# Boese0601/RC-MVSNet

Hardware: AMD Instinct MI355X
Metric: ref-scenes/sec (DTU 3-view 512x640, D=48/32/8) (higher is better)
Workload: dtype f32; 1 GPU; BASELINE configs[1]: CascadeMVSNet_eval.forward, DTU-shaped 3 views 512x640, D=(48,32,8), batch 1 per GPU, fp32, random-init seeded weights; views=3, height=512, width=640, parallelism=scene-per-gpu x1, ranks=1, procs_per_gpu=1, rccl_ranks=0

## Files before the change

rc_mvsnet_amd/_lib.py:

```python
import ast
import ctypes
import os
import re
import subprocess

_HERE = os.path.dirname(os.path.abspath(__file__))
LIB_PATH = os.path.join(_HERE, "librcmvs_hip.so")
CSRC = os.path.join(_HERE, "csrc")
HEADER = os.path.join(os.path.dirname(_HERE), "include", "rcmvs.h")
EXT_HEADERS = (os.path.join(CSRC, "pc_register.h"), os.path.join(CSRC, "view_select.h"), os.path.join(CSRC, "undistort.h"),
               os.path.join(CSRC, "tsdf_mesh.h"), os.path.join(CSRC, "tsdf_sparse.h"), os.path.join(CSRC, "mesh_clean.h"),
               os.path.join(CSRC, "mesh_decimate.h"), os.path.join(CSRC, "mesh_holes.h"))

_lib = None


class RcmvsError(RuntimeError):
    pass


_CTYPES = {"int": ctypes.c_int, "float": ctypes.c_float, "double": ctypes.c_double, "long long": ctypes.c_longlong}


def _const_expr(text):
    def ev(node):
        if isinstance(node, ast.Constant) and type(node.value) is int:
            return node.value
        if isinstance(node, ast.BinOp) and isinstance(node.op, ast.LShift):
            return ev(node.left) << ev(node.right)
        raise ValueError(text)
    return ev(ast.parse(text.strip(), mode="eval").body)


def _ctype(decl, what, c_type):
    if c_type not in _CTYPES:
        raise RcmvsError(f"{HEADER}: `{decl}`: {what} type `{c_type}` is outside the ABI's types ({', '.join(_CTYPES)}, pointers)")
    return _CTYPES[c_type]


def parse_header(text):
    text = re.sub(r"/\*.*?\*/|//[^\n]*", " ", text, flags=re.S)
    signatures, restypes, constants, code = {}, {}, {}, []
    for line in text.splitlines():
        if not line.lstrip().startswith("#"):
            code.append(line)
            continue
        m = re.match(r"\s*#\s*define\s+(RCMVS_\w+)\s+(\S.*)", line)
        if m:
            try:
                value = _const_expr(m.group(2))
            except (ValueError, SyntaxError):
                raise RcmvsError(f"{HEADER}: `{line.strip()}`: not an integer expression of literals, << and parentheses") from None
            if m.group(1) in constants:
                raise RcmvsError(f"{HEADER}: {m.group(1)} is defined twice")
            constants[m.group(1)] = value
    for decl in re.sub(r'extern\s+"C"\s*\{', " ", "\n".join(code)).split(";"):
        decl = " ".join(decl.split())
        if "rcmvs_" not in decl:
            continue
        m = re.fullmatch(r"([\w\s*]+?)\s*\b(rcmvs_\w+)\s*\(([^()]*)\)", decl)
        if not m:
            raise RcmvsError(f"{HEADER}: `{decl}` is not a complete `<type> rcmvs_name(<parameters>);` declaration")
        ret, name, params = m.group(1), m.group(2), m.group(3).strip()
        if name in signatures:
            raise RcmvsError(f"{HEADER}: {name} is declared twice")
# ... 117 lines not shown
```

rc_mvsnet_amd/casmvsnet.py:

```python
import os

FP16_PAIR_DEFAULT = True
ONE_BY_ONE_MFMA = os.environ.get("RCMVS_1X1_MFMA", "1") != "0"
HEAD_PAIR = os.environ.get("RCMVS_HEAD_PAIR", "1") != "0"
CONV11_PROB = int(os.environ.get("RCMVS_CONV11_PROB", "1"))
CONV_TILE = os.environ.get("RCMVS_CONV_TILE", "1") != "0"
CONV_STEM = os.environ.get("RCMVS_CONV_STEM", "1") != "0"
CONV_PAIR = os.environ.get("RCMVS_CONV_PAIR", "1") != "0"
DEEP_PAIR = os.environ.get("RCMVS_DEEP_PAIR", "1") != "0"

import torch
import torch.nn as nn
import torch.nn.functional as F

from . import ops
from ._lib import RcmvsError


def _nhwc(x):
    x = x.contiguous().float()
    return ops.rgb_to_nhwc4(x) if x.shape[1] == 3 else ops.to_channels_last(x)


def _param(mod, name):
    p = mod._parameters.get(name)
    return p if p is not None else getattr(mod, name)


def _packed_of(module, make):
    w = module.conv.weight
    key = (w.data_ptr(), w._version, str(w.device))
    c = module.__dict__.get("_rcmvs_pack")
    if c is None or c[0] != key:
        c = module.__dict__["_rcmvs_pack"] = (key, make(w.detach()))
    return c[1]


def _affine_of(m):
    if getattr(m, "gn", None) is not None:
        raise RcmvsError(f"{type(m).__name__}: GroupNorm blocks are not provided (the reference builds every block with norm='batch_norm')")
    if m.bn is not None:
        return _bn_fold(m.bn)
    b = m.conv.bias
    if b is None:
        return None, None
    return torch.ones_like(b, dtype=torch.float32), b.detach().float().contiguous()


def _same2(v, n):
    return tuple(v) == (n, n)


def _conv2d_block_cl(m, t):
    conv = m.conv
    K = conv.kernel_size[0]
    st = conv.stride[0]
    if (not _same2(conv.kernel_size, K) or K not in (1, 3, 5) or not _same2(conv.padding, K // 2) or not _same2(conv.stride, st)
            or st not in (1, 2) or not _same2(conv.dilation, 1) or conv.groups != 1 or conv.padding_mode != "zeros"):
        raise RcmvsError(f"Conv2d: only square 1x1 / 3x3 / 5x5 kernels with 'same' zero padding, stride 1 or 2, no dilation or groups "
                         f"(the layers of models/modules.py) run on the HIP path; got {conv}")
# ... 105 lines not shown
                self.out_channels.append(b)
        elif num_stage == 3:
            self.inner1 = nn.Conv2d(b * 2, final_chs, 1, bias=True)
            self.inner2 = nn.Conv2d(b * 1, final_chs, 1, bias=True)
            self.out2 = nn.Conv2d(final_chs, b * 2, 3, padding=1, bias=False)
            self.out3 = nn.Conv2d(final_chs, b, 3, padding=1, bias=False)
            self.out_channels += [b * 2, b]
        elif num_stage == 2:
            self.inner1 = nn.Conv2d(b * 2, final_chs, 1, bias=True)
            self.out2 = nn.Conv2d(final_chs, b, 3, padding=1, bias=False)
            self.out_channels.append(b)

    def hip_plan(self):
        sub = self._modules
        mods = [m for seq in ("conv0", "conv1", "conv2") for m in sub[seq]._modules.values()]
        tens = []
        for m in mods:
            cv, bn = m._modules["conv"], m._modules["bn"]
            bb = bn._buffers
            tens += [_param(cv, "weight"), _param(bn, "weight"), _param(bn, "bias"), bb["running_mean"], bb["running_var"], bb["num_batches_tracked"]]
        unet = self.arch_mode == "unet"
        heads = ["out1"] + (["out2", "out3"] if unet else ["inner1", "out2", "inner2", "out3"])
        extra = [t for n in heads if n in sub for t in (_param(sub[n], "weight"), getattr(sub[n], "bias", None)) if t is not None]
        key = tuple((t.data_ptr(), t._version) for t in tens + extra)
        if getattr(self, "_plan", None) is None or key != self._plan_key:
            plan = {}
            names = ["conv0.0", "conv0.1", "conv1.0", "conv1.1", "conv1.2", "conv2.0", "conv2.1", "conv2.2"]
            for n, m in zip(names, mods):
                pad_to = 4 if m.conv.in_channels == 3 else None
                w = m.conv.weight
                if tuple(w.shape) in ((8, 8, 3, 3), (16, 16, 3, 3), (32, 32, 3, 3)) and m.stride == 1:
                    w3 = w.detach().new_zeros(w.shape[0], w.shape[1], 3, 3, 3)
                    w3[:, :, 1] = w.detach()
                    plan[n] = ("mfma3d", ops.pack_conv3d_weight(w3)) + _bn_fold(m.bn)
                    continue
                if tuple(w.shape) in ((32, 16, 5, 5), (16, 8, 5, 5)) and m.stride == 2:
                    w3 = self._w3(self._w5s2(w.detach())).contiguous()
                    plan[n] = ("s2d_mfma3d", ops.pack_conv3d_weight(w3)) + _bn_fold(m.bn)
                    continue
                plan[n] = (ops.pack_conv2d_weight(w, pad_in_to=pad_to),) + _bn_fold(m.bn) + (m.stride,)
            m11, m12 = mods[3], mods[4]
            if CONV_PAIR and all(tuple(m.conv.weight.shape) == (16, 16, 3, 3) and m.stride == 1 for m in (m11, m12)):
                plan["pair1"] = (ops.pack_conv2d_pair(m11.conv.weight, m12.conv.weight),) + _bn_fold(m11.bn) + _bn_fold(m12.bn)
            m00, m01 = mods[0], mods[1]
            if CONV_STEM and tuple(m00.conv.weight.shape) == (8, 3, 3, 3) and tuple(m01.conv.weight.shape) == (8, 8, 3, 3) and m00.stride == 1 and m01.stride == 1:
                plan["stem"] = (plan["conv0.0"][0],) + _bn_fold(m00.bn) + (ops.pack_conv2d_stem(m01.conv.weight),) + _bn_fold(m01.bn)
            m10 = mods[2]
            if CONV_TILE and tuple(m10.conv.weight.shape) == (16, 8, 5, 5) and m10.stride == 2:
                plan["tile10"] = (ops.pack_conv2d_tile(self._w5s2(m10.conv.weight.detach()).contiguous()),) + _bn_fold(m10.bn)
            for n, m in (("conv2.1", mods[6]), ("conv2.2", mods[7])):
                if CONV_TILE and tuple(m.conv.weight.shape) == (32, 32, 3, 3) and m.stride == 1:
                    plan["tile:" + n] = (ops.pack_conv2d_tile(m.conv.weight),) + _bn_fold(m.bn)
            plan["out1"] = ops.pack_conv2d_weight(self.out1.weight)
            if unet:
                for n in ("out2", "out3")[:self.num_stage - 1]:
                    plan[n] = ops.pack_conv3d_weight(self._w3(getattr(self, n).weight.detach()))
            elif self.num_stage >= 2:
                plan["inner1"] = (ops.pack_conv2d_weight(self.inner1.weight), self.inner1.bias.detach().float().contiguous())
                if tuple(self.out2.weight.shape) == (16, 32, 3, 3):
                    w3 = self.out2.weight.detach().new_zeros(16, 32, 3, 3, 3)
                    w3[:, :, 1] = self.out2.weight.detach()
                    plan["out2"] = ("mfma3d", ops.pack_conv3d_weight(w3))
                    if CONV_TILE:
                        plan["out2t"] = ops.pack_conv2d_tile(self.out2.weight)
                else:
                    plan["out2"] = ops.pack_conv2d_weight(self.out2.weight)
            if self.num_stage == 3 and not unet:
                plan["inner2"] = (ops.pack_conv2d_weight(self.inner2.weight), self.inner2.bias.detach().float().contiguous())
                plan["out3"] = ops.pack_conv2d_weight(self.out3.weight)
                plan["fuse_out3"] = tuple(self.inner2.weight.shape[:2]) == (32, 8) and tuple(self.out3.weight.shape[:2]) == (8, 32)
                if plan["fuse_out3"]:
                    plan["fold_out3"] = ops.pack_fpn_folded(self.inner2.weight, self.inner2.bias, self.out3.weight)
                    if os.environ.get("RCMVS_FPN_MFMA", "1") != "0":
                        plan["fold_out3"] = ops.pack_fpn_folded_mfma(plan["fold_out3"])
            self._plan, self._plan_key = plan, key
        return self._plan

    def forward_cl(self, x, lazy=False):
        p = self.hip_plan()

        def cbr(t, n):
            if "tile:" + n in p and not ops._CONV_IMPL:
                img, sc, sh = p["tile:" + n]
                return ops.conv2d_tile(t, img, sc, sh, relu=True)
            if p[n][0] == "mfma3d":
                _, w3, sc, sh = p[n]
                return ops.conv3d(t.unsqueeze(1), w3, sc, sh, relu=True).squeeze(1)
            if p[n][0] == "s2d_mfma3d":
                if t.shape[1] % 2 or t.shape[2] % 2:
                    raise RcmvsError(f"FeatureNet: image height and width must be multiples of 4 (got a {t.shape[1]}x{t.shape[2]} map "
                                     "at the second stride-2 layer), as the reference's three-level pyramid requires")
                _, w3, sc, sh = p[n]
                if ops._CONV_IMPL:
                    return ops.conv3d(self._s2d(t).contiguous().unsqueeze(1), w3, sc, sh, relu=True).squeeze(1)
                return ops.conv2d_s2d(t, w3, sc, sh, relu=True)
            w, sc, sh, stride = p[n]
            return ops.conv2d(t, w, sc, sh, stride=stride, relu=True)

        w00 = p["conv0.0"][0] if len(p["conv0.0"]) == 4 else None
        if "stem" in p and not ops._CONV_IMPL:
            c0 = ops.conv2d_stem(x.contiguous().float(), *p["stem"])
        else:
            c0 = None
        if c0 is not None:
            pass
        elif w00 is not None and w00.ci == 4 and w00.co == 8 and w00.k == 3 and p["conv0.0"][3] == 1 and not ops._CONV_IMPL:
            w, sc, sh, _ = p["conv0.0"]
            c0 = cbr(ops.conv2d_rgb(x.contiguous().float(), w, sc, sh, relu=True), "conv0.1")
        else:
            c0 = cbr(cbr(ops.rgb_to_nhwc4(x.contiguous().float()), "conv0.0"), "conv0.1")
        if "tile10" in p and not ops._CONV_IMPL and c0.shape[1] % 2 == 0 and c0.shape[2] % 2 == 0:
            c10 = ops.conv2d_tile(c0, p["tile10"][0], p["tile10"][1], p["tile10"][2], relu=True, s2d=True)
        else:
            c10 = cbr(c0, "conv1.0")
        if "pair1" in p and not ops._CONV_IMPL:
            c1 = ops.conv2d_pair(c10, *p["pair1"])
        else:
            c1 = cbr(cbr(c10, "conv1.1"), "conv1.2")
        c2 = cbr(cbr(cbr(c1, "conv2.0"), "conv2.1"), "conv2.2")
        def out1(bound=None, t=c2):
            if tuple(self.out1.weight.shape) == (32, 32, 1, 1) and (bound is not None or ONE_BY_ONE_MFMA):
                return ops.conv1x1(t, p["out1"], ysq_absmax=bound, mfma=ONE_BY_ONE_MFMA), bound is not None
            return ops.conv2d(t, p["out1"]), False
        out = {"stage1": out1}
        plain = lambda f: (lambda bound=None: (f(), False))
        if self.arch_mode == "unet":
            one = lambda t, n: ops.conv3d(t.unsqueeze(1), p[n]).squeeze(1)
            if self.num_stage >= 2:
                intra = self.deconv1.forward_cl(c1, c2)
                out["stage2"] = plain(lambda t=intra: one(t, "out2"))
            if self.num_stage == 3:
                intra = self.deconv2.forward_cl(c0, intra)
                out["stage3"] = plain(lambda t=intra: one(t, "out3"))
            return out if lazy else {k: f()[0] for k, f in out.items()}
        if self.num_stage >= 2:
            intra = ops.conv2d(c1, p["inner1"][0], None, p["inner1"][1], up_add=c2)
            if isinstance(p["out2"], tuple):
                def out2(bound=None, t=intra):
                    keep = bound is not None and not ops._CONV_IMPL
                    if "out2t" in p and not ops._CONV_IMPL:
                        return ops.conv2d_tile(t, p["out2t"], ysq_absmax=bound), keep
                    return ops.conv3d(t.unsqueeze(1), p["out2"][1], y_absmax=bound if keep else None, y_absmax_square=keep).squeeze(1), keep
                out["stage2"] = out2
            else:
                out["stage2"] = plain(lambda t=intra: ops.conv2d(t, p["out2"]))
        if self.num_stage == 3:
            if p.get("fuse_out3") and c0.shape[1] % 2 == 0 and c0.shape[2] % 2 == 0:
                if p.get("fold_out3") is not None:
                    out["stage3"] = (lambda bound=None, a=c0, b=intra: (ops.fpn_out_folded(a, b, p["fold_out3"], ysq_absmax=bound), bound is not None))
                else:
                    out["stage3"] = plain(lambda a=c0, b=intra: ops.fpn_out_fused(a, b, p["inner2"][0], p["inner2"][1], p["out3"]))
            else:
                intra = ops.conv2d(c0, p["inner2"][0], None, p["inner2"][1], up_add=intra)
                out["stage3"] = plain(lambda t=intra: ops.conv2d(t, p["out3"]))
        return out if lazy else {k: f()[0] for k, f in out.items()}

    @staticmethod
    def _w3(w):
        p = (3 - w.shape[-1]) // 2
        return F.pad(w.unsqueeze(2), (p, p, p, p, 1, 1))

    @staticmethod
    def _w5s2(w):
        Co, Ci = w.shape[:2]
        w6 = F.pad(w, (0, 1, 0, 1))
        return w6.reshape(Co, Ci, 3, 2, 3, 2).permute(0, 3, 5, 1, 2, 4).reshape(Co, 4 * Ci, 3, 3)

    @staticmethod
    def _s2d(x):
        N, H, W, C = x.shape
        return x.reshape(N, H // 2, 2, W // 2, 2, C).permute(0, 1, 3, 2, 4, 5).reshape(N, H // 2, W // 2, 4 * C)

    def forward_train_cl(self, x, segments=1):
        from .train_ops import ConvPlainFn, conv_bn_train_w
        if self.arch_mode != "fpn":
            raise RcmvsError("FeatureNet(arch_mode='unet'): the train-mode HIP path covers the shipped 'fpn' pyramid only (the one-plane form of "
                             "its transposed convs would put the discarded plane into the batch statistics)")
        N, _, H, W = x.shape
        if H % 4 or W % 4:
            raise RcmvsError("FeatureNet (training): image height and width must be multiples of 4")
        t = F.pad(x.permute(0, 2, 3, 1), (0, 5)).contiguous()

        def cbr(t, m):
            w = m.conv.weight
            if m.stride == 2:
                t, w = self._s2d(t), self._w5s2(w)
            return conv_bn_train_w(self._w3(w), m.bn, t.unsqueeze(1), relu=True, segments=segments).squeeze(1)

        def plain(t, conv):
# ... 266 lines not shown
            out = {"depth": depth, "photometric_confidence": conf}
            if self.train_variant:
                out["volume_feature_no_ref"] = ops.warp_noref(f_cl, small_cl, rot, trans, planes, D, square_first=True)
            return out
        if _hip_training(self, *features, depth_values):
            from . import train_ops
            f_cl = torch.stack([f.float().permute(0, 2, 3, 1) for f in features], dim=1).contiguous()
            res = ops.WarpVarianceFn.apply(f_cl, rot, trans, planes, D, small_cl)
            var, noref = res if self.train_variant else (res, None)
            x8 = cost_regularization.features_cl_train(var)
            depth, conf = train_ops.ProbDepthHeadFn.apply(x8, cost_regularization.prob.weight, planes)
            out = {"depth": depth, "photometric_confidence": conf}
            if self.train_variant:
                out["volume_feature_no_ref"] = noref
            return out
        _unsupported(self, *features, depth_values)


class _CascadeBase(nn.Module):
    TRAIN_VARIANT = False

    def __init__(self, refine=False, ndepths=[48, 32, 8], depth_interals_ratio=[4, 2, 1], share_cr=False,
                 grad_method="detach", arch_mode="fpn", cr_base_chs=[8, 8, 8]):
        super().__init__()
        if refine:
            raise NotImplementedError("refine=True: the reference's RefineNet is not runnable (models/modules.py:511 calls F.cat)")
        self.refine = refine
        self.share_cr = share_cr
        self.ndepths = ndepths
        self.depth_interals_ratio = depth_interals_ratio
        self.grad_method = grad_method
        self.arch_mode = arch_mode
        self.cr_base_chs = cr_base_chs
        self.num_stage = len(ndepths)
        assert len(ndepths) == len(depth_interals_ratio)
        self.stage_infos = {"stage1": {"scale": 4.0}, "stage2": {"scale": 2.0}, "stage3": {"scale": 1.0}}
        self.feature = FeatureNet(base_channels=8, stride=4, num_stage=self.num_stage, arch_mode=self.arch_mode)
        if self.share_cr:
            self.cost_regularization = CostRegNet(in_channels=self.feature.out_channels, base_channels=8)
        else:
            self.cost_regularization = nn.ModuleList([CostRegNet(in_channels=self.feature.out_channels[i],
                                                                 base_channels=self.cr_base_chs[i])
                                                      for i in range(self.num_stage)])
        self.DepthNet = DepthNet(self.TRAIN_VARIANT)

    def _cr(self, s):
        return self.cost_regularization if self.share_cr else self.cost_regularization[s]

    def _forward_hip(self, imgs, proj_matrices, depth_values, features=None, homographies=None):
        B, V, _, H, W = imgs.shape
        imgs = imgs.float()
        depth_values = depth_values.contiguous().float()
        feats_cl = None
        if features is None:
            feats_cl = self.feature.forward_cl(imgs.reshape(B * V, 3, H, W), lazy=True)
        outputs = {}
        depth = None
        bounds = None
        need_fill = False
        pair = getattr(self, "fp16_pair", None)
        if pair is None:
            pair = FP16_PAIR_DEFAULT if os.environ.get("RCMVS_FP16_PAIR") is None else os.environ["RCMVS_FP16_PAIR"] == "1"
        if pair and B == 1:
            bounds = getattr(self, "_pair_bounds", None)
            if getattr(self, "_is_replica", False):
                bounds = torch.zeros(self.num_stage, CostRegNet.BOUND_ROWS, ops.ABSMAX_FLOATS, device=imgs.device, dtype=torch.float32)
            elif bounds is None or bounds.device != imgs.device:
                bounds = self._pair_bounds = torch.zeros(self.num_stage, CostRegNet.BOUND_ROWS, ops.ABSMAX_FLOATS, device=imgs.device, dtype=torch.float32)
            else:
                need_fill = True
        if homographies is None:
            if self.num_stage <= 4:
                rots, transs = ops.compose_homography_stages([proj_matrices["stage{}".format(k + 1)].contiguous().float() for k in range(self.num_stage)],
                                                             zero=bounds if need_fill else None)
                need_fill = False
            else:
                rt = [ops.compose_homography(proj_matrices["stage{}".format(k + 1)].contiguous().float()) for k in range(self.num_stage)]
                rots, transs = [r for r, _ in rt], [t for _, t in rt]
        if need_fill:
            bounds.zero_()
        for s in range(self.num_stage):
            key = "stage{}".format(s + 1)
            scale = int(self.stage_infos[key]["scale"])
            D = self.ndepths[s]
            bound_kept = False
            if feats_cl is not None:
                fk, bound_kept = feats_cl[key](bounds[s][0] if bounds is not None else None)
                h, w, C = fk.shape[1:]
                f_cl = fk.view(B, V, h, w, C)
            else:
                C, h, w = features[key].shape[1:]
                f_cl = ops.to_channels_last(features[key].contiguous()).view(B, V, h, w, C)
            if homographies is not None:
                rot, trans = homographies[key]
            else:
                rot, trans = rots[s], transs[s]
            planes = ops.hypothesis_planes(depth, depth_values, (H, W), scale, D, self.depth_interals_ratio[s])
            var = ops.warp_variance(f_cl, rot, trans, planes, D, uniform_planes=depth is None)
            cr = self._cr(s)
            vmax = None
            if bounds is not None:
                vmax = bounds[s]
                if not bound_kept:
                    ops.absmax(f_cl, square=True, out=vmax[0])
            plan = cr.hip_plan()
            if vmax is not None and HEAD_PAIR and (CONV11_PROB == 2 or (CONV11_PROB == 1 and D == 8)):
                depth, conf = cr.features_cl(var, vmax, plan, logits=True, planes=planes)
            else:
                x8 = cr.features_cl(var, vmax, plan)
                depth, conf = ops.depth_head(x8, plan["prob"], planes, x_absmax=vmax[CostRegNet.BOUND_ROWS - 1] if vmax is not None and HEAD_PAIR else None)
            out = {"depth": depth, "photometric_confidence": conf}
            if self.TRAIN_VARIANT:
                small_cl = ops.resize_rgb_cl(imgs.reshape(B * V, 3, H, W).contiguous(), (h, w)).view(B, V, h, w, 3)
                out["volume_feature_no_ref"] = ops.warp_noref(f_cl, small_cl, rot, trans, planes, D, square_first=True)
            outputs[key] = out
            outputs.update(out)
        return outputs

    def _forward_train_hip(self, imgs, proj_matrices, depth_values):
        from . import train_ops
        B, V, _, H, W = imgs.shape
        imgs = imgs.float()
        depth_values = depth_values.contiguous().float()
        fv = self.feature.forward_train_cl(imgs.transpose(0, 1).reshape(V * B, 3, H, W), segments=V)
        features = [{k: f[v * B:(v + 1) * B] for k, f in fv.items()} for v in range(V)]
        outputs = {}
        depth = None
        for s in range(self.num_stage):
            key = "stage{}".format(s + 1)
            scale = int(self.stage_infos[key]["scale"])
            D = self.ndepths[s]
            f_cl = torch.stack([f[key] for f in features], dim=1).contiguous()
            h, w = f_cl.shape[2:4]
# ... 46 lines not shown
```

rc_mvsnet_amd/csrc/conv2d_tile.hip:

```cpp
#include "common.h"
#include "x3_pieces.h"
#include <atomic>

namespace rcmvs {

constexpr int T2_TH = 8, T2_TW = 32;
constexpr int T2_IH = T2_TH + 2, T2_IW = T2_TW + 2;
constexpr int T2_CI = 32, T2_PB = T2_CI * 2;
constexpr int T2_IPL = T2_IH * T2_IW * T2_PB;
constexpr int T2_LDS = 3 * T2_IPL + 64;
constexpr int T2_KS = 9;
constexpr long long t2_img_halfs(int co) { return (long long)T2_KS * 3 * (co / 16) * 64 * 8; }
__device__ __forceinline__ int t2_swz(int c) { return ((c >> 2) & 1) * 32; }

long long conv2d_tile_weight_floats(int co) { return (co == 16 || co == 32) ? t2_img_halfs(co) / 2 : 0; }

__global__ void conv2d_tile_pack_kernel(const float* __restrict__ w, unsigned short* __restrict__ img, int MT) {
    const int t = blockIdx.x * blockDim.x + threadIdx.x;
    if (t >= T2_KS * MT * 64 * 8) return;
    const int e = t & 7, lane = (t >> 3) & 63, mt = (t >> 9) % MT, j = (t >> 9) / MT;
    const int co = mt * 16 + (lane & 15), ci = (lane >> 4) * 8 + e;
    const float v = w[(co * T2_CI + ci) * 9 + j];
    const unsigned hb = __float_as_uint(v) & 0xffff0000u;
    const float r1 = v - __uint_as_float(hb);
    const unsigned mb = __float_as_uint(r1) & 0xffff0000u;
    const float r2 = r1 - __uint_as_float(mb);
    const unsigned lb = __float_as_uint(r2) & 0xffff0000u;
    const long long base = (((long long)j * 3) * MT + mt) * 512 + lane * 8 + e;
    img[base] = (unsigned short)(hb >> 16);
    img[base + MT * 512] = (unsigned short)(mb >> 16);
    img[base + 2 * MT * 512] = (unsigned short)(lb >> 16);
}

template <bool S2D, int CO>
__global__ __launch_bounds__(CO * 16, CO == 16 ? 2 : 1) void conv2d_tile_kernel(
    const float* __restrict__ x, const x3_u32x4* __restrict__ wimg, const float* __restrict__ scale, const float* __restrict__ shift,
    float* __restrict__ y, int H, int W, int tiles_w, int relu, float* __restrict__ ysq) {
    extern __shared__ __attribute__((aligned(16))) x3_byte smem[];
    x3_byte* const ib = smem;
    float* const redmax = reinterpret_cast<float*>(smem + 3 * T2_IPL);
    constexpr int OOB = 0x7ffffff0;
    const int tid = threadIdx.x, lane = tid & 63;
    const int wave = __builtin_amdgcn_readfirstlane(tid >> 6);
    const int n = lane & 15, kk = lane >> 4;
    constexpr int MT = CO / 16, NW = 4 * MT, NHALF = MT;
    const int mt = MT == 2 ? (wave & 1) : 0, rg = MT == 2 ? (wave >> 1) : wave;
    const int view = blockIdx.y;
    const unsigned t2 = xcd_remap(blockIdx.x, gridDim.x);
    const int tw = t2 % tiles_w, th = t2 / tiles_w;
    const int h0 = th * T2_TH, w0 = tw * T2_TW;
    __amdgpu_buffer_rsrc_t xrs = __builtin_amdgcn_make_buffer_rsrc(const_cast<float*>(x + (long long)view * H * W * T2_CI), (short)0, H * W * T2_CI * 4, 0x00020000);
    auto offset_of = [&](int r, int c, int c4) -> int {
        const int ih = h0 - 1 + r, iw = w0 - 1 + c;
        if (!(ih >= 0 && ih < H && iw >= 0 && iw < W)) return OOB;
// ... 55 lines not shown
            for (int t = 0; t < 2; ++t) a1[t] = x3_mfma<3>(A[j][1], bh[t], a1[t]);
#pragma unroll
            for (int t = 0; t < 2; ++t) a2[t] = x3_mfma<3>(A[j][2], bh[t], a2[t]);
#pragma unroll
            for (int t = 0; t < 2; ++t) a2[t] = x3_mfma<3>(A[j][1], bm[t], a2[t]);
        }
#pragma unroll
        for (int t = 0; t < 2; ++t) {
            x3_f32x4 v = (a0[t] + (a1[t] + a2[t])) * sc + sh;
            if (relu) v = __builtin_elementwise_max(v, (x3_f32x4){0.f, 0.f, 0.f, 0.f});
            const int oh = h0 + row, ow = w0 + 16 * t + n;
            if (oh < H && ow < W) {
                *reinterpret_cast<x3_f32x4*>(yb + ((long long)oh * W + ow) * CO + co0) = v;
                vmax = x3_absmax4(vmax, v);
            }
        }
    }
    if (ysq) {
#pragma unroll
        for (int m = 32; m > 0; m >>= 1) vmax = fmaxf(vmax, __shfl_xor(vmax, m));
        if (lane == 0) redmax[wave] = vmax;
        __syncthreads();
        if (tid == 0) {
            float m = redmax[0];
#pragma unroll
            for (int i = 1; i < NW; ++i) m = fmaxf(m, redmax[i]);
            atomicMax(reinterpret_cast<unsigned int*>(ysq) + ((blockIdx.x + blockIdx.y * gridDim.x) & 63) * 16, __float_as_uint(m * m));
        }
    }
}

int conv2d_tile_launch(const float* x, const float* wimg, const float* scale, const float* shift, float* y, int N, int H, int W, int Co, int s2d, int relu,
                       float* ysq, hipStream_t st) {
    if ((long long)H * W * T2_CI * 4 >= 0x7ffffff0LL || N > 65535) return fail(-1, "conv2d_tile: map too large for 32-bit offsets");
    if (!(Co == 16 || (Co == 32 && !s2d))) return fail(-1, "conv2d_tile: built for 32 -> 16 (plain or space-to-depth) and 32 -> 32 (got Co=%d s2d=%d)", Co, s2d);
    static std::atomic<bool> raised[64];
    int dev = 0;
    if (hipGetDevice(&dev) != hipSuccess || dev < 0 || dev >= 64) return fail(-1, "conv2d_tile: cannot query the device");
    if (!raised[dev].load(std::memory_order_acquire)) {
        if (hipFuncSetAttribute((const void*)conv2d_tile_kernel<false, 16>, hipFuncAttributeMaxDynamicSharedMemorySize, T2_LDS) != hipSuccess ||
            hipFuncSetAttribute((const void*)conv2d_tile_kernel<true, 16>, hipFuncAttributeMaxDynamicSharedMemorySize, T2_LDS) != hipSuccess ||
            hipFuncSetAttribute((const void*)conv2d_tile_kernel<false, 32>, hipFuncAttributeMaxDynamicSharedMemorySize, T2_LDS) != hipSuccess)
            return fail(-1, "conv2d_tile: cannot raise the dynamic LDS limit to %d bytes", T2_LDS);
        raised[dev].store(true, std::memory_order_release);
    }
    const int tw_ = (W + T2_TW - 1) / T2_TW, th_ = (H + T2_TH - 1) / T2_TH;
    const x3_u32x4* wi = reinterpret_cast<const x3_u32x4*>(wimg);
    if (Co == 32) hipLaunchKernelGGL((conv2d_tile_kernel<false, 32>), dim3(tw_ * th_, N), dim3(512), T2_LDS, st, x, wi, scale, shift, y, H, W, tw_, relu, ysq);
    else if (s2d) hipLaunchKernelGGL((conv2d_tile_kernel<true, 16>), dim3(tw_ * th_, N), dim3(256), T2_LDS, st, x, wi, scale, shift, y, H, W, tw_, relu, ysq);
    else hipLaunchKernelGGL((conv2d_tile_kernel<false, 16>), dim3(tw_ * th_, N), dim3(256), T2_LDS, st, x, wi, scale, shift, y, H, W, tw_, relu, ysq);
    return launch_status("conv2d_tile");
}

}

using namespace rcmvs;

extern "C" {

long long rcmvs_conv2d_tile_weight_floats(int Co) { return conv2d_tile_weight_floats(Co); }

int rcmvs_pack_conv2d_tile(const float* w, float* image, int Co, void* stream) {
    RCMVS_REQUIRE(w && image, "pack_conv2d_tile: null pointer");
    RCMVS_REQUIRE(Co == 16 || Co == 32, "pack_conv2d_tile: built for 16 or 32 output channels (got %d)", Co);
    hipLaunchKernelGGL(conv2d_tile_pack_kernel, dim3((T2_KS * (Co / 16) * 64 * 8 + 255) / 256), dim3(256), 0, as_stream(stream), w, reinterpret_cast<unsigned short*>(image), Co / 16);
    return launch_status("pack_conv2d_tile");
}

int rcmvs_conv2d_tile_fwd(const float* x, const float* image, const float* scale, const float* shift, float* y, int N, int H, int W, int Co, int s2d, int relu,
                          float* ysq_absmax, void* stream) {
    RCMVS_REQUIRE(x && image && y, "conv2d_tile_fwd: null pointer");
    RCMVS_REQUIRE(N > 0 && H > 0 && W > 0, "conv2d_tile_fwd: bad sizes");
    return conv2d_tile_launch(x, image, scale, shift, y, N, H, W, Co, s2d, relu, ysq_absmax, as_stream(stream));
}

}
```

rc_mvsnet_amd/ops.py:

```python
import ctypes
import os

import torch

from . import _lib

K1_EVENTS = None
K1_UNIFORM_PLANES = _lib.CONSTANTS["RCMVS_K1_UNIFORM_PLANES"]
K1_FAST_BLEND = _lib.CONSTANTS["RCMVS_K1_FAST_BLEND"]
CONV_EVENTS = None


_FIRST_STREAM = {}


def _multi_stream_allowed():
    return os.environ.get("GPU_MAX_HW_QUEUES") == "1" or os.environ.get("RCMVS_ALLOW_MULTI_STREAM") == "1"


def _stream():
    st = torch.cuda.current_stream()
    key = st.device_index
    first = _FIRST_STREAM.setdefault(key, st.cuda_stream)
    if first != st.cuda_stream and not _multi_stream_allowed():
# ... 329 lines not shown
    if up_add is not None and tuple(up_add.shape) != (N, Ho // 2, Wo // 2, Co):
        raise _lib.RcmvsError(f"conv2d: up_add {tuple(up_add.shape)} does not match half of the output {tuple(y.shape)}")
    _lib.call("rcmvs_conv2d_fwd", _chk(x, "x"), _chk(w_packed.blob, "w"), _opt(scale, "scale"), _opt(shift, "shift"),
              _opt(up_add, "up_add"), _chk(y, "y"), N, H, W, Ci, Co, K, stride, int(relu), _stream())
    return y


def conv1x1(x, w_packed, scale=None, shift=None, up_add=None, relu=False, ysq_absmax=None, mfma=False):
    N, H, W, Ci = x.shape
    Co = w_packed.co
    if w_packed.ci != Ci or w_packed.k != 1:
        raise _lib.RcmvsError(f"conv1x1: input has {Ci} channels, weight is {w_packed.ci} -> {Co} with k={w_packed.k}")
    if up_add is not None and tuple(up_add.shape) != (N, H // 2, W // 2, Co):
        raise _lib.RcmvsError(f"conv1x1: up_add {tuple(up_add.shape)} does not match half of the output")
    y = torch.empty((N, H, W, Co), device=x.device, dtype=torch.float32)
    _lib.call("rcmvs_conv1x1_mfma_fwd" if mfma else "rcmvs_conv1x1_fwd", _chk(x, "x"), _chk(w_packed.blob, "w"), _opt(scale, "scale"), _opt(shift, "shift"),
              _opt(up_add, "up_add"), _chk(y, "y"), _opt(ysq_absmax, "ysq_absmax"), N, H, W, Ci, Co, int(relu), _stream())
    return y


def conv2d_rgb(x, w_packed, scale=None, shift=None, relu=False):
    N, C, H, W = x.shape
    if C != 3 or w_packed.ci != 4 or w_packed.co != 8 or w_packed.k != 3:
        raise _lib.RcmvsError(f"conv2d_rgb: expected a (N,3,H,W) input and a 3 -> 8 3x3 weight packed to 4 input channels (got {tuple(x.shape)}, {w_packed.ci} -> {w_packed.co}, k={w_packed.k})")
    y = torch.empty((N, H, W, 8), device=x.device, dtype=torch.float32)
    _lib.call("rcmvs_conv2d_fwd", _chk(x, "x"), _chk(w_packed.blob, "w"), _opt(scale, "scale"), _opt(shift, "shift"), None,
              _chk(y, "y"), N, H, W, 3, 8, 3, 1, int(relu), _stream())
    return y


def pack_conv2d_tile(w):
    Co = w.shape[0]
    if Co not in (16, 32) or tuple(w.shape) != (Co, 32, 3, 3):
        raise _lib.RcmvsError("pack_conv2d_tile: built for 32 -> 16 and 32 -> 32 3x3 layers")
    lib = _lib.load()
    img = torch.empty(int(lib.rcmvs_conv2d_tile_weight_floats(Co)), device=w.device, dtype=torch.float32)
    _lib.call("rcmvs_pack_conv2d_tile", _chk(w.detach().float().contiguous(), "w"), _chk(img, "image"), Co, _stream())
    return img


def conv2d_tile(x, image, scale=None, shift=None, relu=False, s2d=False, ysq_absmax=None):
    N, Hx, Wx, C = x.shape
    lib = _lib.load()
    Co = {int(lib.rcmvs_conv2d_tile_weight_floats(c)): c for c in (16, 32)}.get(image.numel())
    if Co is None or C != (8 if s2d else 32) or (s2d and (Hx % 2 or Wx % 2 or Co != 16)):
        raise _lib.RcmvsError(f"conv2d_tile: unexpected input {tuple(x.shape)} (s2d={s2d}) or image of {image.numel()} floats")
    H, W = (Hx // 2, Wx // 2) if s2d else (Hx, Wx)
    y = torch.empty((N, H, W, Co), device=x.device, dtype=torch.float32)
    _lib.call("rcmvs_conv2d_tile_fwd", _chk(x, "x"), _chk(image, "image"), _opt(scale, "scale"), _opt(shift, "shift"), _chk(y, "y"), N, H, W, Co, int(s2d), int(relu),
              _opt(ysq_absmax, "ysq_absmax"), _stream())
    return y


def pack_conv2d_stem(wb):
    if tuple(wb.shape) != (8, 8, 3, 3):
        raise _lib.RcmvsError("pack_conv2d_stem: built for an 8 -> 8 3x3 second layer")
    lib = _lib.load()
    img = torch.empty(int(lib.rcmvs_conv2d_stem_weight_floats()), device=wb.device, dtype=torch.float32)
    _lib.call("rcmvs_pack_conv2d_stem", _chk(wb.detach().float().contiguous(), "wb"), _chk(img, "image"), _stream())
    return img


def conv2d_stem(x, w_a_packed, scale_a, shift_a, image_b, scale_b, shift_b):
    N, C, H, W = x.shape
    if C != 3 or w_a_packed.ci != 4 or w_a_packed.co != 8 or w_a_packed.k != 3:
        raise _lib.RcmvsError(f"conv2d_stem: expected a (N,3,H,W) input and a 3 -> 8 3x3 weight packed to 4 input channels (got {tuple(x.shape)}, {w_a_packed.ci} -> {w_a_packed.co}, k={w_a_packed.k})")
    y = torch.empty((N, H, W, 8), device=x.device, dtype=torch.float32)
    _lib.call("rcmvs_conv2d_stem_fwd", _chk(x, "x"), _chk(w_a_packed.blob, "w_a"), _chk(scale_a, "scale_a"), _chk(shift_a, "shift_a"), _chk(image_b, "image_b"),
              _chk(scale_b, "scale_b"), _chk(shift_b, "shift_b"), _chk(y, "y"), N, H, W, _stream())
    return y


def fpn_out_fused(lat, up, w_inner_packed, b_inner, w_out_packed):
    N, H, W, CL = lat.shape
    CM, CO = w_inner_packed.co, w_out_packed.co
    if w_inner_packed.ci != CL or w_inner_packed.k != 1 or w_out_packed.ci != CM or w_out_packed.k != 3:
        raise _lib.RcmvsError("fpn_out_fused: expected a 1x1 lateral conv followed by a 3x3 output conv on matching channels")
    if tuple(up.shape) != (N, H // 2, W // 2, CM):
        raise _lib.RcmvsError(f"fpn_out_fused: up {tuple(up.shape)} does not match half of {tuple(lat.shape)} with {CM} channels")
    y = torch.empty((N, H, W, CO), device=lat.device, dtype=torch.float32)
    _lib.call("rcmvs_fpn_out_fused", _chk(lat, "lat"), _chk(up, "up"), _chk(w_inner_packed.blob, "w_inner"), _chk(b_inner, "b_inner"),
              _chk(w_out_packed.blob, "w_out"), _chk(y, "y"), N, H, W, CL, CM, CO, _stream())
    return y


FPN_FOLDED_FLOATS = _lib.CONSTANTS["RCMVS_FPN_FOLDED_FLOATS"]


def pack_fpn_folded(w_inner, b_inner, w_out):
    wi = w_inner.detach().double().reshape(32, 8)
    wo = w_out.detach().double()
    b = b_inner.detach().double()
    wb = torch.einsum("mi,omyx->yxio", wi, wo)
    bt = torch.einsum("m,omyx->yxo", b, wo)
    inside = {0: (1, 2), 1: (0, 1, 2), 2: (0, 1)}
    bs = torch.stack([torch.stack([sum(bt[ky, kx] for ky in inside[cy] for kx in inside[cx]) for cx in range(3)]) for cy in range(3)])
    rows = lambda p: ((0,), (1, 2)) if p == 0 else ((0, 1), (2,))
    wa = torch.zeros(2, 2, 2, 2, 32, 8, dtype=torch.float64, device=wo.device)
    for py in range(2):
        for px in range(2):
            for ry in range(2):
                for rx in range(2):
                    for ky in rows(py)[ry]:
                        for kx in rows(px)[rx]:
                            wa[py, px, ry, rx] += wo[:, :, ky, kx].t()
    tab = torch.cat((wb.reshape(-1), bs.reshape(-1), wa.reshape(-1))).float().contiguous()
# ... 158 lines not shown
```

Measured before the change: 940.4 ref-scenes/s.

## Fuse conv2.2, out1 1x1 conv and inner1 lateral upsample-add into one kernel

Adds a conv2d_tail HIP kernel that computes the last 3x3 conv of the FPN trunk, then uses the tile kept in LDS to run the out1 1x1 conv (MFMA with a 3-way bf16 split) and the inner1 lateral 1x1 conv plus nearest-upsample add. It writes c2, out1 and intra in one launch and also folds in the absmax bound reduction. Feature extraction is moved after the bounds buffer is allocated so the bound can be passed in. This removes two launches and the re-reads of c2 from global memory, at the cost of higher register and LDS pressure and extra shape checks.

```diff
diff --git a/rc_mvsnet_amd/_lib.py b/rc_mvsnet_amd/_lib.py
--- a/rc_mvsnet_amd/_lib.py
+++ b/rc_mvsnet_amd/_lib.py
@@ -10,7 +10,7 @@
 HEADER = os.path.join(os.path.dirname(_HERE), "include", "rcmvs.h")
 EXT_HEADERS = (os.path.join(CSRC, "pc_register.h"), os.path.join(CSRC, "view_select.h"), os.path.join(CSRC, "undistort.h"),
                os.path.join(CSRC, "tsdf_mesh.h"), os.path.join(CSRC, "tsdf_sparse.h"), os.path.join(CSRC, "mesh_clean.h"),
-               os.path.join(CSRC, "mesh_decimate.h"), os.path.join(CSRC, "mesh_holes.h"))
+               os.path.join(CSRC, "mesh_decimate.h"), os.path.join(CSRC, "mesh_holes.h"), os.path.join(CSRC, "conv2d_tail.h"))
 
 _lib = None
 
diff --git a/rc_mvsnet_amd/casmvsnet.py b/rc_mvsnet_amd/casmvsnet.py
--- a/rc_mvsnet_amd/casmvsnet.py
+++ b/rc_mvsnet_amd/casmvsnet.py
@@ -6,6 +6,7 @@
 CONV11_PROB = int(os.environ.get("RCMVS_CONV11_PROB", "1"))
 CONV_TILE = os.environ.get("RCMVS_CONV_TILE", "1") != "0"
 CONV_STEM = os.environ.get("RCMVS_CONV_STEM", "1") != "0"
+CONV_TAIL = os.environ.get("RCMVS_CONV_TAIL", "1") != "0"
 CONV_PAIR = os.environ.get("RCMVS_CONV_PAIR", "1") != "0"
 DEEP_PAIR = os.environ.get("RCMVS_DEEP_PAIR", "1") != "0"
 
@@ -217,6 +218,8 @@
                 if CONV_TILE and tuple(m.conv.weight.shape) == (32, 32, 3, 3) and m.stride == 1:
                     plan["tile:" + n] = (ops.pack_conv2d_tile(m.conv.weight),) + _bn_fold(m.bn)
             plan["out1"] = ops.pack_conv2d_weight(self.out1.weight)
+            plan["tail"] = (CONV_TILE and CONV_TAIL and ONE_BY_ONE_MFMA and not unet and self.num_stage >= 2 and "tile:conv2.2" in plan
+                            and tuple(self.out1.weight.shape) == (32, 32, 1, 1) and tuple(self.inner1.weight.shape) == (32, 16, 1, 1))
             if unet:
                 for n in ("out2", "out3")[:self.num_stage - 1]:
                     plan[n] = ops.pack_conv3d_weight(self._w3(getattr(self, n).weight.detach()))
@@ -241,7 +244,7 @@
             self._plan, self._plan_key = plan, key
         return self._plan
 
-    def forward_cl(self, x, lazy=False):
+    def forward_cl(self, x, lazy=False, bound=None):
         p = self.hip_plan()
 
         def cbr(t, n):
@@ -282,8 +285,18 @@
             c1 = ops.conv2d_pair(c10, *p["pair1"])
         else:
             c1 = cbr(cbr(c10, "conv1.1"), "conv1.2")
-        c2 = cbr(cbr(cbr(c1, "conv2.0"), "conv2.1"), "conv2.2")
-        def out1(bound=None, t=c2):
+        c21 = cbr(cbr(c1, "conv2.0"), "conv2.1")
+        o1 = intra = None
+        if p["tail"] and not ops._CONV_IMPL and c1.shape[1] == 2 * c21.shape[1] and c1.shape[2] == 2 * c21.shape[2]:
+            img, sc, sh = p["tile:conv2.2"]
+            c2, o1, intra = ops.conv2d_tail(c21, img, sc, sh, p["out1"], c1, p["inner1"][0], p["inner1"][1], relu=True, ysq_absmax=bound)
+        else:
+            c2 = cbr(c21, "conv2.2")
+        def out1(bound=None, t=c2, trunk_bound=bound):
+            if o1 is not None:
+                if bound is not None and (trunk_bound is None or bound.data_ptr() != trunk_bound.data_ptr()):
+                    ops.absmax(o1, square=True, out=bound)
+                return o1, bound is not None
             if tuple(self.out1.weight.shape) == (32, 32, 1, 1) and (bound is not None or ONE_BY_ONE_MFMA):
                 return ops.conv1x1(t, p["out1"], ysq_absmax=bound, mfma=ONE_BY_ONE_MFMA), bound is not None
             return ops.conv2d(t, p["out1"]), False
@@ -299,7 +312,8 @@
                 out["stage3"] = plain(lambda t=intra: one(t, "out3"))
             return out if lazy else {k: f()[0] for k, f in out.items()}
         if self.num_stage >= 2:
-            intra = ops.conv2d(c1, p["inner1"][0], None, p["inner1"][1], up_add=c2)
+            if intra is None:
+                intra = ops.conv2d(c1, p["inner1"][0], None, p["inner1"][1], up_add=c2)
             if isinstance(p["out2"], tuple):
                 def out2(bound=None, t=intra):
                     keep = bound is not None and not ops._CONV_IMPL
@@ -672,8 +686,6 @@
         imgs = imgs.float()
         depth_values = depth_values.contiguous().float()
         feats_cl = None
-        if features is None:
-            feats_cl = self.feature.forward_cl(imgs.reshape(B * V, 3, H, W), lazy=True)
         outputs = {}
         depth = None
         bounds = None
@@ -699,6 +711,8 @@
                 rots, transs = [r for r, _ in rt], [t for _, t in rt]
         if need_fill:
             bounds.zero_()
+        if features is None:
+            feats_cl = self.feature.forward_cl(imgs.reshape(B * V, 3, H, W), lazy=True, bound=bounds[0][0] if bounds is not None else None)
         for s in range(self.num_stage):
             key = "stage{}".format(s + 1)
             scale = int(self.stage_infos[key]["scale"])
diff --git a/rc_mvsnet_amd/csrc/conv2d_tail.h b/rc_mvsnet_amd/csrc/conv2d_tail.h
--- /dev/null
+++ b/rc_mvsnet_amd/csrc/conv2d_tail.h
@@ -0,0 +1,13 @@
+#ifndef RCMVS_CONV2D_TAIL_H
+#define RCMVS_CONV2D_TAIL_H
+#ifdef __cplusplus
+extern "C" {
+#endif
+
+int rcmvs_conv2d_tail_fwd(const float* x, const float* image, const float* scale, const float* shift, const float* w_out1, const float* c1, const float* w_inner1,
+                          const float* bias_inner1, float* y, float* y_out1, float* y_intra, int N, int H, int W, int relu, float* ysq_absmax, void* stream);
+
+#ifdef __cplusplus
+}
+#endif
+#endif
diff --git a/rc_mvsnet_amd/csrc/conv2d_tile.hip b/rc_mvsnet_amd/csrc/conv2d_tile.hip
--- a/rc_mvsnet_amd/csrc/conv2d_tile.hip
+++ b/rc_mvsnet_amd/csrc/conv2d_tile.hip
@@ -1,5 +1,6 @@
 #include "common.h"
 #include "x3_pieces.h"
+#include "conv2d_tail.h"
 #include <atomic>
 
 namespace rcmvs {
@@ -161,6 +162,247 @@
     return launch_status("conv2d_tile");
 }
 
+constexpr int TL_TH = 4, TL_IH = TL_TH + 2;
+constexpr int TL_IPL = TL_IH * T2_IW * T2_PB;
+constexpr int TL_STR = 36;
+constexpr int TL_TRB = 64 * TL_STR * 4;
+constexpr int TL_SCR = TL_TH * TL_TRB > 3 * TL_IPL ? TL_TH * TL_TRB : 3 * TL_IPL;
+constexpr int TL_C2 = TL_TH * T2_TW * TL_STR * 4;
+constexpr int TL_LDS = TL_SCR + TL_C2 + 64;
+
+__global__ __launch_bounds__(64 * TL_TH, 2) void conv2d_tail_kernel(
+    const float* __restrict__ x, const x3_u32x4* __restrict__ wimg, const float* __restrict__ scale, const float* __restrict__ shift, float* __restrict__ y,
+    const float* __restrict__ w1, float* __restrict__ y1, float* __restrict__ ysq,
+    const float* __restrict__ c1, const float* __restrict__ wl, const float* __restrict__ bl, float* __restrict__ intra,
+    int H, int W, int tiles_w, int relu) {
+    extern __shared__ __attribute__((aligned(16))) x3_byte smem[];
+    x3_byte* const ib = smem;
+    float* const c2t = reinterpret_cast<float*>(smem + TL_SCR);
+    float* const redmax = reinterpret_cast<float*>(smem + TL_SCR + TL_C2);
+    constexpr int OOB = 0x7ffffff0;
+    constexpr int CO = 32, MT = 2, NHALF = 1;
+    const int tid = threadIdx.x, lane = tid & 63;
+    const int wave = __builtin_amdgcn_readfirstlane(tid >> 6);
+    const int n = lane & 15, kk = lane >> 4;
+    const int mt = wave & 1, rg = wave >> 1;
+    const int view = blockIdx.y;
+    const unsigned t2 = xcd_remap(blockIdx.x, gridDim.x);
+    const int tw = t2 % tiles_w, th = t2 / tiles_w;
+    const int h0 = th * TL_TH, w0 = tw * T2_TW;
+    __amdgpu_buffer_rsrc_t xrs = __builtin_amdgcn_make_buffer_rsrc(const_cast<float*>(x + (long long)view * H * W * T2_CI), (short)0, H * W * T2_CI * 4, 0x00020000);
+    auto offset_of = [&](int r, int c, int c4) -> int {
+        const int ih = h0 - 1 + r, iw = w0 - 1 + c;
+        if (!(ih >= 0 && ih < H && iw >= 0 && iw < W)) return OOB;
+        return ((ih * W + iw) * T2_CI + c4 * 4) * 4;
+    };
+    constexpr int NR = TL_IH / NHALF;
+    x3_u32x4 pf[NR + 1];
+    const int lc = (tid & 255) >> 3, l4 = tid & 7, r0 = tid >> 8;
+#pragma unroll
+    for (int r = 0; r < NR; ++r) pf[r] = __builtin_amdgcn_raw_buffer_load_b128(xrs, offset_of(r0 + r * NHALF, lc, l4), 0, 0);
+    const int er = tid >> 4, ec = 32 + ((tid >> 3) & 1);
+    pf[NR] = __builtin_amdgcn_raw_buffer_load_b128(xrs, tid < TL_IH * 16 ? offset_of(er, ec, l4) : OOB, 0, 0);
+    x3_u32x4 A[T2_KS][3];
+#pragma unroll
+    for (int j = 0; j < T2_KS; ++j)
+#pragma unroll
+        for (int p = 0; p < 3; ++p) A[j][p] = wimg[((j * 3 + p) * MT + mt) * 64 + lane];
+    const int co0 = mt * 16 + 4 * kk;
+    const x3_f32x4 sc = scale ? *reinterpret_cast<const x3_f32x4*>(scale + co0) : (x3_f32x4){1.f, 1.f, 1.f, 1.f};
+    const x3_f32x4 sh = shift ? *reinterpret_cast<const x3_f32x4*>(shift + co0) : (x3_f32x4){0.f, 0.f, 0.f, 0.f};
+    const int trow = wave, qh = h0 + trow;
+    __amdgpu_buffer_rsrc_t crs = __builtin_amdgcn_make_buffer_rsrc(const_cast<float*>(c1 + (long long)view * H * W * 64), (short)0, H * W * 256, 0x00020000);
+    x3_f32x4 cv[2][4];
+    {
+        const int ox = 2 * w0 + lane;
+        const bool in = qh < H && ox < 2 * W;
+#pragma unroll
+        for (int r = 0; r < 2; ++r)
+#pragma unroll
+            for (int q = 0; q < 4; ++q)
+                cv[r][q] = __builtin_bit_cast(x3_f32x4, __builtin_amdgcn_raw_buffer_load_b128(crs, in ? (((2 * qh + r) * (2 * W) + ox) * 16 + q * 4) * 4 : OOB, 0, 0));
+    }
+    float w1v[2][8];
+#pragma unroll
+    for (int m = 0; m < 2; ++m)
+#pragma unroll
+        for (int i = 0; i < 8; ++i) w1v[m][i] = w1[(kk * 8 + i) * CO + m * 16 + n];
+    auto park = [&](x3_u32x4 v, int r, int c) {
+        x3_u32x2 h, m, l;
+        x3_split4(__builtin_bit_cast(x3_f32x4, v), h, m, l);
+        x3_byte* q = ib + (r * T2_IW + c) * T2_PB + ((l4 * 8) ^ t2_swz(c));
+        *reinterpret_cast<x3_u32x2*>(q) = h;
+        *reinterpret_cast<x3_u32x2*>(q + TL_IPL) = m;
+        *reinterpret_cast<x3_u32x2*>(q + 2 * TL_IPL) = l;
+    };
+#pragma unroll
+    for (int r = 0; r < NR; ++r) park(pf[r], r0 + r * NHALF, lc);
+    if (tid < TL_IH * 16) park(pf[NR], er, ec);
+    __syncthreads();
+    float* yb = y + (long long)view * H * W * CO;
+#pragma unroll 1
+    for (int rr = 0; rr < 2; ++rr) {
+        const int row = 2 * rg + rr;
+        x3_f32x4 a0[2], a1[2], a2[2];
+#pragma unroll
+        for (int t = 0; t < 2; ++t) a0[t] = a1[t] = a2[t] = (x3_f32x4){0.f, 0.f, 0.f, 0.f};
+#pragma unroll
+        for (int j = 0; j < T2_KS; ++j) {
+            const int dy = j / 3, dx = j - 3 * dy;
+            x3_u32x4 bh[2], bm[2], bl3[2];
+#pragma unroll
+            for (int t = 0; t < 2; ++t) {
+                const int c = 16 * t + n + dx;
+                const x3_byte* q = ib + ((row + dy) * T2_IW + c) * T2_PB + ((kk * 16) ^ t2_swz(c));
+                bh[t] = *reinterpret_cast<const x3_u32x4*>(q); bm[t] = *reinterpret_cast<const x3_u32x4*>(q + TL_IPL); bl3[t] = *reinterpret_cast<const x3_u32x4*>(q + 2 * TL_IPL);
+            }
+#pragma unroll
+            for (int t = 0; t < 2; ++t) a0[t] = x3_mfma<3>(A[j][0], bh[t], a0[t]);
+#pragma unroll
+            for (int t = 0; t < 2; ++t) a1[t] = x3_mfma<3>(A[j][0], bm[t], a1[t]);
+#pragma unroll
+            for (int t = 0; t < 2; ++t) a2[t] = x3_mfma<3>(A[j][0], bl3[t], a2[t]);
+#pragma unroll
+            for (int t = 0; t < 2; ++t) a1[t] = x3_mfma<3>(A[j][1], bh[t], a1[t]);
+#pragma unroll
+            for (int t = 0; t < 2; ++t) a2[t] = x3_mfma<3>(A[j][2], bh[t], a2[t]);
+#pragma unroll
+            for (int t = 0; t < 2; ++t) a2[t] = x3_mfma<3>(A[j][1], bm[t], a2[t]);
+        }
+#pragma unroll
+        for (int t = 0; t < 2; ++t) {
+            x3_f32x4 v = (a0[t] + (a1[t] + a2[t])) * sc + sh;
+            if (relu) v = __builtin_elementwise_max(v, (x3_f32x4){0.f, 0.f, 0.f, 0.f});
+            const int oh = h0 + row, ow = w0 + 16 * t + n;
+            if (oh < H && ow < W) *reinterpret_cast<x3_f32x4*>(yb + ((long long)oh * W + ow) * CO + co0) = v;
+            *reinterpret_cast<x3_f32x4*>(c2t + (row * T2_TW + 16 * t + n) * TL_STR + co0) = v;
+        }
+    }
+    __syncthreads();
+    {
+        x3_u32x4 A1[2][3];
+#pragma unroll
+        for (int m = 0; m < 2; ++m) {
+            unsigned hb[8], mb[8], lb[8];
+#pragma unroll
+            for (int i = 0; i < 8; ++i) {
+                const float v = w1v[m][i];
+                hb[i] = __float_as_uint(v) & 0xffff0000u;
+                const float r1 = v - __uint_as_float(hb[i]);
+                mb[i] = __float_as_uint(r1) & 0xffff0000u;
+                const float r2 = r1 - __uint_as_float(mb[i]);
+                lb[i] = __float_as_uint(r2) & 0xffff0000u;
+            }
+#pragma unroll
+            for (int j = 0; j < 4; ++j) {
+                A1[m][0][j] = (hb[2 * j] >> 16) | hb[2 * j + 1];
+                A1[m][1][j] = (mb[2 * j] >> 16) | mb[2 * j + 1];
+                A1[m][2][j] = (lb[2 * j] >> 16) | lb[2 * j + 1];
+            }
+        }
+        float* y1b = y1 + (long long)view * H * W * CO;
+        float vmax = 0.0f;
+#pragma unroll
+        for (int t = 0; t < 2; ++t) {
+            const float* src = c2t + (trow * T2_TW + 16 * t + n) * TL_STR + 8 * kk;
+            x3_u32x2 hA, mA, lA, hB, mB, lB;
+            x3_split4(*reinterpret_cast<const x3_f32x4*>(src), hA, mA, lA);
+            x3_split4(*reinterpret_cast<const x3_f32x4*>(src + 4), hB, mB, lB);
+            const x3_u32x4 bq[3] = {(x3_u32x4){hA.x, hA.y, hB.x, hB.y}, (x3_u32x4){mA.x, mA.y, mB.x, mB.y}, (x3_u32x4){lA.x, lA.y, lB.x, lB.y}};
+            const int ow = w0 + 16 * t + n;
+            const bool live = qh < H && ow < W;
+#pragma unroll
+            for (int m = 0; m < 2; ++m) {
+                x3_f32x4 acc[3] = {(x3_f32x4){0.f, 0.f, 0.f, 0.f}, (x3_f32x4){0.f, 0.f, 0.f, 0.f}, (x3_f32x4){0.f, 0.f, 0.f, 0.f}};
+                acc[2] = x3_mfma<3>(A1[m][0], bq[2], acc[2]);
+                acc[1] = x3_mfma<3>(A1[m][0], bq[1], acc[1]);
+                acc[0] = x3_mfma<3>(A1[m][0], bq[0], acc[0]);
+                acc[2] = x3_mfma<3>(A1[m][1], bq[1], acc[2]);
+                acc[1] = x3_mfma<3>(A1[m][1], bq[0], acc[1]);
+                acc[2] = x3_mfma<3>(A1[m][2], bq[0], acc[2]);
+                const x3_f32x4 v = acc[0] + (acc[1] + acc[2]);
+                if (live) {
+                    *reinterpret_cast<x3_f32x4*>(y1b + ((long long)qh * W + ow) * CO + m * 16 + 4 * kk) = v;
+                    vmax = x3_absmax4(vmax, v);
+                }
+            }
+        }
+        if (ysq) {
+#pragma unroll
+            for (int m = 32; m > 0; m >>= 1) vmax = fmaxf(vmax, __shfl_xor(vmax, m));
+            if (lane == 0) redmax[wave] = vmax;
+        }
+    }
+    {
+        float acc[2][CO];
+#pragma unroll
+        for (int r = 0; r < 2; ++r)
+#pragma unroll
+            for (int co = 0; co < CO; ++co) acc[r][co] = 0.0f;
+#pragma unroll 1
+        for (int c4 = 0; c4 < 4; ++c4) {
+            const float* wt = wl + c4 * 4 * CO;
+#pragma unroll
+            for (int j = 0; j < 4; ++j)
+#pragma unroll
+                for (int co = 0; co < CO; ++co)
+#pragma unroll
+                    for (int r = 0; r < 2; ++r) acc[r][co] = fmaf(cv[r][0][j], wt[j * CO + co], acc[r][co]);
+#pragma unroll
+            for (int r = 0; r < 2; ++r) { cv[r][0] = cv[r][1]; cv[r][1] = cv[r][2]; cv[r][2] = cv[r][3]; }
+        }
+        const float* upp = c2t + (trow * T2_TW + (lane >> 1)) * TL_STR;
+        float* trb = reinterpret_cast<float*>(smem + wave * TL_TRB);
+        float* ib2 = intra + (long long)view * H * W * 4 * CO;
+#pragma unroll
+        for (int r = 0; r < 2; ++r) {
+            if (r) __builtin_amdgcn_wave_barrier();
+#pragma unroll
+            for (int co = 0; co < CO; co += 4) {
+                const x3_f32x4 u4 = *reinterpret_cast<const x3_f32x4*>(upp + co);
+                x3_f32x4 v;
+                v.x = u4.x + (acc[r][co] + bl[co]); v.y = u4.y + (acc[r][co + 1] + bl[co + 1]);
+                v.z = u4.z + (acc[r][co + 2] + bl[co + 2]); v.w = u4.w + (acc[r][co + 3] + bl[co + 3]);
+                *reinterpret_cast<x3_f32x4*>(trb + lane * TL_STR + co) = v;
+            }
+            __builtin_amdgcn_wave_barrier();
+            const long long rowbase = ((long long)(2 * qh + r) * (2 * W) + 2 * w0) * CO;
+#pragma unroll
+            for (int i = 0; i < CO / 4; ++i) {
+                const int e = i * 64 + lane, px = e >> 3, q = e & 7;
+                const x3_f32x4 v = *reinterpret_cast<const x3_f32x4*>(trb + px * TL_STR + q * 4);
+                if (qh < H && 2 * w0 + px < 2 * W) *reinterpret_cast<x3_f32x4*>(ib2 + rowbase + px * CO + q * 4) = v;
+            }
+        }
+    }
+    if (ysq) {
+        __syncthreads();
+        if (tid == 0) {
+            float m = redmax[0];
+#pragma unroll
+            for (int i = 1; i < TL_TH; ++i) m = fmaxf(m, redmax[i]);
+            atomicMax(reinterpret_cast<unsigned int*>(ysq) + ((blockIdx.x + blockIdx.y * gridDim.x) & 63) * 16, __float_as_uint(m * m));
+        }
+    }
+}
+
+int conv2d_tail_launch(const float* x, const float* wimg, const float* scale, const float* shift, float* y, const float* w1, float* y1, float* ysq,
+                       const float* c1, const float* wl, const float* bl, float* intra, int N, int H, int W, int relu, hipStream_t st) {
+    if ((long long)H * W * 256 >= 0x7ffffff0LL || N > 65535) return fail(-1, "conv2d_tail: map too large for 32-bit offsets");
+    static std::atomic<bool> raised[64];
+    int dev = 0;
+    if (hipGetDevice(&dev) != hipSuccess || dev < 0 || dev >= 64) return fail(-1, "conv2d_tail: cannot query the device");
+    if (!raised[dev].load(std::memory_order_acquire)) {
+        if (hipFuncSetAttribute((const void*)conv2d_tail_kernel, hipFuncAttributeMaxDynamicSharedMemorySize, TL_LDS) != hipSuccess)
+            return fail(-1, "conv2d_tail: cannot raise the dynamic LDS limit to %d bytes", TL_LDS);
+        raised[dev].store(true, std::memory_order_release);
+    }
+    const int tw_ = (W + T2_TW - 1) / T2_TW, th_ = (H + TL_TH - 1) / TL_TH;
+    hipLaunchKernelGGL(conv2d_tail_kernel, dim3(tw_ * th_, N), dim3(64 * TL_TH), TL_LDS, st, x, reinterpret_cast<const x3_u32x4*>(wimg), scale, shift, y, w1, y1, ysq,
+                       c1, wl, bl, intra, H, W, tw_, relu);
+    return launch_status("conv2d_tail");
+}
+
 }
 
 using namespace rcmvs;
@@ -183,4 +425,11 @@
     return conv2d_tile_launch(x, image, scale, shift, y, N, H, W, Co, s2d, relu, ysq_absmax, as_stream(stream));
 }
 
-}
+int rcmvs_conv2d_tail_fwd(const float* x, const float* image, const float* scale, const float* shift, const float* w_out1, const float* c1, const float* w_inner1,
+                          const float* bias_inner1, float* y, float* y_out1, float* y_intra, int N, int H, int W, int relu, float* ysq_absmax, void* stream) {
+    RCMVS_REQUIRE(x && image && w_out1 && c1 && w_inner1 && bias_inner1 && y && y_out1 && y_intra, "conv2d_tail_fwd: null pointer");
+    RCMVS_REQUIRE(N > 0 && H > 0 && W > 0, "conv2d_tail_fwd: bad sizes");
+    return conv2d_tail_launch(x, image, scale, shift, y, w_out1, y_out1, ysq_absmax, c1, w_inner1, bias_inner1, y_intra, N, H, W, relu, as_stream(stream));
+}
+
+}
diff --git a/rc_mvsnet_amd/ops.py b/rc_mvsnet_amd/ops.py
--- a/rc_mvsnet_amd/ops.py
+++ b/rc_mvsnet_amd/ops.py
@@ -405,6 +405,22 @@
     return y
 
 
+def conv2d_tail(x, image, scale, shift, w_out1, c1, w_inner1, bias_inner1, relu=True, ysq_absmax=None):
+    N, H, W, C = x.shape
+    lib = _lib.load()
+    if C != 32 or image.numel() != int(lib.rcmvs_conv2d_tile_weight_floats(32)) or tuple(c1.shape) != (N, 2 * H, 2 * W, 16):
+        raise _lib.RcmvsError(f"conv2d_tail: unexpected inputs {tuple(x.shape)}, {tuple(c1.shape)} or image of {image.numel()} floats")
+    if (w_out1.ci, w_out1.co, w_out1.k) != (32, 32, 1) or (w_inner1.ci, w_inner1.co, w_inner1.k) != (16, 32, 1) or bias_inner1.numel() != 32:
+        raise _lib.RcmvsError("conv2d_tail: built for a 32 -> 32 1x1 output conv and a 16 -> 32 1x1 lateral conv with bias")
+    c2 = torch.empty((N, H, W, 32), device=x.device, dtype=torch.float32)
+    o1 = torch.empty((N, H, W, 32), device=x.device, dtype=torch.float32)
+    intra = torch.empty((N, 2 * H, 2 * W, 32), device=x.device, dtype=torch.float32)
+    _lib.call("rcmvs_conv2d_tail_fwd", _chk(x, "x"), _chk(image, "image"), _opt(scale, "scale"), _opt(shift, "shift"), _chk(w_out1.blob, "w_out1"), _chk(c1, "c1"),
+              _chk(w_inner1.blob, "w_inner1"), _chk(bias_inner1, "bias_inner1"), _chk(c2, "y"), _chk(o1, "y_out1"), _chk(intra, "y_intra"), N, H, W, int(relu),
+              _opt(ysq_absmax, "ysq_absmax"), _stream())
+    return c2, o1, intra
+
+
 def pack_conv2d_stem(wb):
     if tuple(wb.shape) != (8, 8, 3, 3):
         raise _lib.RcmvsError("pack_conv2d_stem: built for an 8 -> 8 3x3 second layer")
```

Result: no change. 944.1 ref-scenes/s (median of 6 runs) (+0.4%).
